# FraPria/proovread

Hardware: AMD Instinct MI355X
Metric: corrected long-read Mbases/sec per node (higher is better)
Workload: dtype int32

## Files before the change

### proovread_amd/csrc/seed_api.cpp

```cpp
#include <algorithm>
#include <climits>
#include <cstdio>
#include <cstdlib>
#include <cstring>
#include <vector>

#include "ctx.h"
#include "seed_index_dev.h"
#include "seed_plan.h"

static int seed_text4(pr_ctx *c, seedc::IndexView &v, hipStream_t s) {
    int rc = c->sd[SI_TEXT4].ensure((size_t)ix_pack4_words(v.n_text) * 8);
    if (rc) return rc;
    const int e = ix_pack4_launch(v.text, v.n_text, c->sd[SI_TEXT4].as<uint64_t>(), s);
    if (e) return set_error(PR_ERR_HIP, "text packing: %s", hipGetErrorString((hipError_t)e));
    v.text4 = c->sd[SI_TEXT4].as<uint64_t>();
    v.walk_nw = v.n_text > ((int64_t)64 << 24) ? 1 : 4;
    if (const char *w = getenv("PRGPU_SEED_WALK_NW"))
        v.walk_nw = atoi(w) == 1 ? 1 : 4;
    return 0;
}

static int upload_blk_fr(pr_ctx *c, seedc::IndexView &v, const int64_t *cstart, const int64_t *off, int n_lr,
                         int64_t l_pac, int64_t n_text, hipStream_t s) {
// ... 241 lines not shown
    seed_digest_tables(text, koff, kpos, kext, cnt, cstart, cblk, lro, ksplit, out6);
    return 0;
}

extern "C" int pr_seed_gpu_index_koff(pr_ctx *c, uint64_t *koff, uint64_t *ksplit) {
    if (!c || !koff) return set_error(PR_ERR_ARG, "null arg");
    if (!c->seed_loaded) return set_error(PR_ERR_ARG, "no device seed index");
    HIPCHK(hipSetDevice(c->device));
    HIPCHK(hipStreamSynchronize(c->stream));
    HIPCHK(hipMemcpy(koff, c->seed_view.koff, ((size_t)seedc::NK + 1) * 8, hipMemcpyDeviceToHost));
    if (ksplit && c->seed_view.ksplit)
        HIPCHK(hipMemcpy(ksplit, c->seed_view.ksplit, (size_t)seedc::NK * 8, hipMemcpyDeviceToHost));
    return 0;
}

extern "C" int pr_seed_gpu_index_last_ms(pr_ctx *c, double *ms) {
    if (!c || !ms) return set_error(PR_ERR_ARG, "null arg");
    *ms = c->ms_index;
    return 0;
}

extern "C" int pr_srset_load(pr_ctx *c, int64_t n_sr, const int64_t *off, const uint8_t *seq) {
    if (!c || n_sr < 0 || !off || (off[n_sr] && !seq) || off[0] != 0) return set_error(PR_ERR_ARG, "bad arg");
    HIPCHK(hipSetDevice(c->device));
    int rc = upload(c->ls[LS_SRSEQ], seq, (size_t)off[n_sr], c->stream);
    if (rc) return rc;
    HIPCHK(hipStreamSynchronize(c->stream));
    c->ss_off.assign(off, off + n_sr + 1);
    c->ss_samp_off.clear();
    c->ls[LS_SRSAMP].release();
    return 0;
}

static int gather_ranges(pr_ctx *c, const int64_t *ranges, int n_ranges, int64_t max_reads, DevBuf &dst,
                         std::vector<int64_t> &off) {
    if (c->ss_off.empty()) return set_error(PR_ERR_ARG, "no resident short reads (pr_srset_load)");
    const int64_t N = (int64_t)c->ss_off.size() - 1;
    off.assign(1, 0);
    for (int k = 0; k < n_ranges; ++k) {
        const int64_t r0 = ranges[2 * k], r1 = ranges[2 * k + 1];
        if (r0 < 0 || r1 < r0 || r1 > N) return set_error(PR_ERR_ARG, "record range outside the short reads");
        for (int64_t i = r0; i < r1; ++i) off.push_back(off.back() + c->ss_off[(size_t)i + 1] - c->ss_off[(size_t)i]);
    }
    if ((int64_t)off.size() - 1 > max_reads) return set_error(PR_ERR_CAPACITY, "too many short reads in one sample");
    HIPCHK(hipSetDevice(c->device));
    int rc = dst.ensure((size_t)off.back() + 1);
    if (rc) return rc;
    std::vector<int64_t> so, dn, ln;
    int64_t at = 0;
    for (int k = 0; k < n_ranges; ++k) {
        const int64_t b0 = c->ss_off[(size_t)ranges[2 * k]], b1 = c->ss_off[(size_t)ranges[2 * k + 1]];
        if (b1 > b0) {
            if (!so.empty() && so.back() + ln.back() == b0) ln.back() += b1 - b0;
            else so.push_back(b0), dn.push_back(at), ln.push_back(b1 - b0);
        }
        at += b1 - b0;
    }
    const int e = sr_gather_launch(c->ls[LS_SRSEQ].as<uint8_t>(), dst.as<uint8_t>(), so.data(), dn.data(), ln.data(),
                                   (int64_t)so.size(), (void *)c->stream);
    if (e) return set_error(PR_ERR_HIP, "short-read gather: %s", hipGetErrorString((hipError_t)e));
    return 0;
}

extern "C" int pr_srset_sample(pr_ctx *c, const int64_t *ranges, int n_ranges) {
    if (!c || n_ranges < 0 || (n_ranges && !ranges)) return set_error(PR_ERR_ARG, "null arg");
    std::vector<int64_t> off;
    int rc = gather_ranges(c, ranges, n_ranges, INT64_MAX, c->ls[LS_SRSAMP], off);
    if (rc) return rc;
    c->ss_samp_off.swap(off);
    return 0;
}

namespace {

struct SeedMap {
    pr_ctx *c;
    hipStream_t s;
    DevBuf *D;
    int n_sr;
    int qmax;
    SeedDev K;
    seedc::Caps small, caps;
    int64_t waves;
    int64_t lanes2;
    int64_t chunk;
    int32_t budget;
    std::vector<int32_t> nout, st;
    std::vector<int64_t> pre;
    int64_t total = 0, bad = 0;
    int32_t bad_flags = 0;
};

void map_plan(SeedMap &M, const pr_seed_opts *o, const int64_t *sr_off) {
    pr_ctx *c = M.c;
    int qmax = 1;
    for (int i = 0; i < M.n_sr; ++i) qmax = std::max<int>(qmax, (int)(sr_off[i + 1] - sr_off[i]));
    M.qmax = qmax;
    seedc::Caps &caps = M.caps, &small = M.small;
    caps = seedc::device_caps(qmax);
    caps.hi = c->seed_view.ksplit != nullptr;
    caps.nopos = 1;
    small = seedc::device_caps_small(std::min(qmax, caps.lmax));
    small.hi = caps.hi;
    small.nopos = 1;
    small.lazy = seedc::lazy_occ(*o) ? 1 : 0;
    if (const char *sc = getenv("PRGPU_SEED_SMALL"))
        sscanf(sc, "%d,%d,%d,%d,%d", &small.hits, &small.iv, &small.mems, &small.seeds, &small.chains);
    M.budget = small.lazy ? seedp::PASS1_LAZY_BUDGET : 0;
    if (const char *bu = getenv("PRGPU_SEED_BUDGET")) M.budget = small.lazy ? std::max(0, atoi(bu)) : 0;
    SeedDev &K = M.K;
    K = SeedDev{};
    K.V = c->seed_view;
    K.O = *o;
    K.n_sr = M.n_sr;
    K.caps = small;
    K.stride = seedc::scratch_bytes(small);
    const char *wpc = getenv("PRGPU_SEED_WAVES_PER_CU");
    size_t fr = 0, tot = 0;
    (void)hipMemGetInfo(&fr, &tot);
    (void)hipGetLastError();
    const int per_cu = wpc ? atoi(wpc) : 16;
    const int64_t full = caps.hi ? 0 : (int64_t)c->n_cu * per_cu * 64 * K.stride;
    M.waves = seedp::pass1_waves(M.n_sr, c->n_cu, per_cu, getenv("PRGPU_SEED_BALANCE") != nullptr,
                                 seedp::pass1_budget((int64_t)fr, (int64_t)M.D[SB_SCRATCH].cap, full), K.stride);
    K.n_lanes = M.waves;
    M.lanes2 = (int64_t)c->n_cu * seed_slots_per_cu(c->seed_view.walk_nw);
    const char *ob = getenv("PRGPU_SEED_OUT_MB");
    M.chunk = seedp::out_chunk(ob ? std::max<int64_t>(1, atoll(ob)) << 20
                                  : seedp::out_budget((int64_t)fr, (int64_t)M.D[SB_OUT].cap),
                               (int64_t)caps.out * (int64_t)sizeof(pr_seed_task));
}

int map_buffers(SeedMap &M, const pr_seed_opts *o, const uint8_t *sr_seq, bool in_sb_seq, const int64_t *sr_off) {
    pr_ctx *c = M.c;
    DevBuf *D = M.D;
    SeedDev &K = M.K;
    const int n_sr = M.n_sr;
    hipStream_t s = M.s;
    int rc;
    K.dp = nullptr;
    if (seedc::seed_flt_min_score(*o, M.qmax) >= 0) {
        if ((rc = D[SB_DP].ensure((size_t)M.waves * 2 * 201 * 64 * sizeof(int16_t)))) return rc;
        K.dp = D[SB_DP].as<int16_t>();
    }
    const int64_t scratch = std::max<int64_t>(M.waves * 64 * K.stride, M.lanes2 * seedc::scratch_bytes(M.caps));
    const int64_t nb = n_sr ? sr_off[n_sr] : 0;
    const int64_t slot_bytes = (int64_t)M.caps.out * (int64_t)sizeof(pr_seed_task);
    c->seed_sr_bases = nb;
    if ((!in_sb_seq && (rc = upload(D[SB_SEQ], sr_seq, (size_t)nb, s))) || (rc = upload(D[SB_OFF], sr_off, (size_t)n_sr + 1, s)) ||
        (rc = D[SB_SCRATCH].ensure((size_t)scratch)) ||
        (rc = D[SB_OUT].ensure((size_t)(std::min<int64_t>(M.chunk, n_sr) * slot_bytes + 16))) ||
        (rc = D[SB_NOUT].ensure((size_t)n_sr * 4 + 16)) || (rc = D[SB_STATUS].ensure((size_t)n_sr * 4 + 16)) ||
        (rc = D[SB_NEXT].ensure(256)) || (rc = D[SB_PRE].ensure(((size_t)n_sr + 1) * 8)) ||
        (rc = D[SB_DENSE].ensure(sizeof(pr_seed_task))))
        return rc;
    K.sr_seq = D[SB_SEQ].as<uint8_t>();
    K.sr_off = D[SB_OFF].as<int64_t>();
    K.out = D[SB_OUT].as<pr_seed_task>();
    K.n_out = D[SB_NOUT].as<int32_t>();
    K.status = D[SB_STATUS].as<int32_t>();
    K.next = D[SB_NEXT].as<int32_t>();
    K.prof = reinterpret_cast<unsigned long long *>(D[SB_NEXT].as<uint8_t>() + 64);
    HIPCHK(hipMemsetAsync(K.next, 0, 256, s));
    return 0;
}

int pass1(SeedMap &M, int64_t r0, int64_t r1, std::vector<int32_t> &redo, seedp::Flagged &f) {
    DevBuf *D = M.D;
    SeedDev &K = M.K;
    hipStream_t s = M.s;
    int rc;
    K.caps = M.small;
    K.caps.budget = M.budget;
    K.stride = seedc::scratch_bytes(M.small);
    K.n_lanes = M.waves;
    K.batch = 64;
    K.scratch = D[SB_SCRATCH].as<uint8_t>();
    K.rlist = nullptr;
    K.n_list = 0;
    K.out0 = r0;
    K.n_sr = r1;
    int32_t start = (int32_t)r0;
    const char *lpt = getenv("PRGPU_SEED_LPT");
    if (lpt && lpt[0] == '1') {
        int32_t *order = nullptr;
        if ((rc = D[SB_ORDER].ensure(seed_order_bytes(r1 - r0)))) return rc;
        int eo = seed_order_launch(K, r0, r1 - r0, D[SB_ORDER].p, &order, (void *)s);
        if (eo) return set_error(PR_ERR_HIP, "seed order: %s", hipGetErrorString((hipError_t)eo));
        K.rlist = order;
        K.n_list = r1 - r0;
        start = 0;
    }
    HIPCHK(hipMemcpyAsync(K.next, &start, 4, hipMemcpyHostToDevice, s));
    int e = seed_batch_launch(K, (void *)s);
    if (e) return set_error(PR_ERR_HIP, "seed kernel: %s", hipGetErrorString((hipError_t)e));
    if (r0 == 0) HIPCHK(hipEventRecord(M.c->ev[10], s));
    std::vector<int32_t> st1((size_t)(r1 - r0)), no1((size_t)(r1 - r0));
    if ((rc = download(st1.data(), D[SB_STATUS], (size_t)(r1 - r0), s, (size_t)r0)) ||
        (rc = download(no1.data(), D[SB_NOUT], (size_t)(r1 - r0), s, (size_t)r0)))
        return rc;
    HIPCHK(hipStreamSynchronize(s));
    for (int64_t i = r0; i < r1; ++i)
        if (st1[(size_t)(i - r0)]) {
            redo.push_back((int32_t)i);
            f.add(st1[(size_t)(i - r0)], no1[(size_t)(i - r0)]);
        }
    return 0;
}

int launch_pass(SeedMap &M, const char *name, bool by_wave, const seedc::Caps &caps, int64_t lanes,
                const std::vector<int32_t> &reads, int batch = 64) {
    SeedDev &K = M.K;
    K.caps = caps;
    K.stride = seedc::scratch_bytes(caps);
    K.n_lanes = lanes;
    K.batch = batch;
    K.scratch = M.D[SB_SCRATCH].as<uint8_t>();
    K.rlist = M.D[SB_PRE].as<int32_t>();
    K.n_list = (int64_t)reads.size();
    HIPCHK(hipMemcpyAsync(M.D[SB_PRE].p, reads.data(), reads.size() * 4, hipMemcpyHostToDevice, M.s));
    HIPCHK(hipMemsetAsync(K.next, 0, 4, M.s));
    const int e = by_wave ? seed_launch(K, (void *)M.s) : seed_batch_launch(K, (void *)M.s);
    if (e) return set_error(PR_ERR_HIP, "seed kernel (%s): %s", name, hipGetErrorString((hipError_t)e));
    return 0;
}

int still_flagged(SeedMap &M, int64_t r0, int64_t r1, const std::vector<int32_t> &reads, std::vector<int32_t> &left,
                  int32_t &flags) {
    std::vector<int32_t> st((size_t)(r1 - r0));
    int rc = download(st.data(), M.D[SB_STATUS], (size_t)(r1 - r0), M.s, (size_t)r0);
    if (rc) return rc;
    HIPCHK(hipStreamSynchronize(M.s));
    left.clear();
    flags = 0;
    for (int32_t i : reads)
        if (st[(size_t)(i - r0)]) left.push_back(i), flags |= st[(size_t)(i - r0)];
    return 0;
}

int pass1b(SeedMap &M, int64_t r0, int64_t r1, const seedp::Flagged &f, std::vector<int32_t> &redo, seedc::Caps &p2caps,
           bool &p2_ran) {
    if (!seedp::pass1b_wanted(f)) return 0;
    const seedp::Pass1bCaps p = seedp::pass1b_caps(M.small, M.caps, f);
    DevBuf &scr = M.D[SB_SCRATCH];
    int rc;
    size_t fr = 0, tot = 0;
    (void)hipMemGetInfo(&fr, &tot);
    (void)hipGetLastError();
    if (const int64_t want = seedp::pass1b_scratch_want(M.waves, f.n, p.sb, (int64_t)fr, (int64_t)scr.cap)) {
        HIPCHK(hipStreamSynchronize(M.s));
        if ((rc = scr.ensure((size_t)want))) return rc;
    }
    const char *p1b = getenv("PRGPU_SEED_1B");
    const seedp::Pass1bForce force =
        !p1b ? seedp::P1B_AUTO : !strcmp(p1b, "wave") ? seedp::P1B_FORCE_WAVE : seedp::P1B_FORCE_LANE;
    const seedp::Pass1bRun r =
        seedp::pass1b_run(p, f, M.small.hits, force, (int64_t)scr.cap, M.waves, M.lanes2, M.c->n_cu);
    if (r.mode == seedp::P1B_SKIP) return 0;
    const bool by_wave = r.mode == seedp::P1B_WAVE;
    seedp::Pass1bBatch b{64, r.wb};
    if (!by_wave && p.cb.lazy) {
        const char *bb = getenv("PRGPU_SEED_1B_BATCH");
        b = seedp::pass1b_batch(r, f.n, M.waves, (int64_t)scr.cap, p.sb, bb ? atoi(bb) : 0);
    }
    if ((rc = launch_pass(M, by_wave ? "pass 1b, waves" : "pass 1b", by_wave, by_wave ? p.cw : p.cb, by_wave ? r.ww : b.waves,
                          redo, b.batch)))
        return rc;
    M.c->seed_pass_reads[by_wave ? 1 : 0] += (int64_t)redo.size();
    if (by_wave) p2caps = p.cw, p2_ran = true;
    std::vector<int32_t> left;
    int32_t fl;
    if ((rc = still_flagged(M, r0, r1, redo, left, fl))) return rc;
    redo.swap(left);
    M.K.rlist = nullptr;
    M.K.n_list = 0;
    return 0;
}

int pass2_and_later(SeedMap &M, int64_t r0, int64_t r1, std::vector<int32_t> &redo, seedc::Caps cg, bool p2_ran) {
    if (redo.empty()) return 0;
    int rc;
    if (!p2_ran) {
        if ((rc = launch_pass(M, "pass 2", true, M.caps, std::min<int64_t>(M.lanes2, (int64_t)redo.size()), redo))) return rc;
        HIPCHK(hipStreamSynchronize(M.s));
        M.c->seed_pass_reads[2] += (int64_t)redo.size();
    }
    for (int pass = 3; pass <= 6; ++pass) {
        std::vector<int32_t> again;
        int32_t fl;
        if ((rc = still_flagged(M, r0, r1, redo, again, fl))) return rc;
        if (again.empty() || (fl & (seedc::SC_OVER_LEN | seedc::SC_OVER_OUT))) break;
        cg = seedc::grow_caps(cg, fl, 4);
        redo.swap(again);
        const int64_t lanes = std::min<int64_t>(M.lanes2, (int64_t)redo.size());
        if ((rc = M.D[SB_SCRATCH].ensure((size_t)(lanes * seedc::scratch_bytes(cg))))) return rc;
        char name[16];
        snprintf(name, sizeof name, "pass %d", pass);
        if ((rc = launch_pass(M, name, true, cg, lanes, redo))) return rc;
        HIPCHK(hipStreamSynchronize(M.s));
// ... 185 lines not shown
```

### proovread_amd/csrc/seed_core.h

```cpp
#pragma once
#include <math.h>
#include <stdint.h>

#include "../../include/prgpu.h"

#if defined(__HIPCC__)
#define SC_HD __host__ __device__ inline
#else
#define SC_HD inline
#endif

#if defined(PR_SEED_STATS) && !defined(__HIP_DEVICE_COMPILE__)
extern unsigned long long pr_seed_stat_g[24];
#define SC_STAT(k, v) __atomic_fetch_add(&pr_seed_stat_g[k], (unsigned long long)(v), __ATOMIC_RELAXED)
#else
#define SC_STAT(k, v) ((void)0)
#endif

namespace prgpu {
namespace seedc {

constexpr int KI = 12;
constexpr uint32_t NK = 1u << (2 * KI);
constexpr int KX = 28;
// ... 1179 lines not shown
    for (int ci = 0; ci < nch; ++ci) {
        const Chain &c = S.ch[ci];
        if (c.kept == 0) continue;
        const bool rev = S.seeds[c.head].rbeg >= I.l_pac;
        const int64_t L = I.lr_off[c.rid + 1] - I.lr_off[c.rid];
        const int64_t cs = rev ? I.l_pac + (I.l_pac - I.lr_off[c.rid + 1]) : I.lr_off[c.rid];
        if (no + c.n > cap_out) return SC_OVER_OUT;
        const int first = no;
        int idx = 0;
        int64_t r0 = INT64_MAX, r1 = INT64_MIN;
        for (int32_t k = c.head; k >= 0; k = S.seeds[k].nx) {
            const Seed &s = S.seeds[k];
            int score = s.len;
            if (flt >= 0) {
                const int x = scores ? scores[k]
                                     : (dp16 ? seed_sw_score(I, O, q, len, s, c.rid, dp16, dp16 + 201 * 64, 64)
                                             : seed_sw_score(I, O, q, len, s, c.rid, swH, swE));
                if (x >= 0 && x < flt) continue;
                score = x < 0 ? s.len * O.a : x;
            }
            const int64_t b = s.rbeg - (s.qbeg + cal_max_gap(O, s.qbeg));
            const int64_t e = s.rbeg + s.len + ((len - s.qbeg - s.len) + cal_max_gap(O, len - s.qbeg - s.len));
            r0 = r0 < b ? r0 : b;
            r1 = r1 > e ? r1 : e;
            pr_seed_task &t = out[no];
            t.sr = sid;
            t.lr = c.rid;
            t.strand = rev ? 1 : 0;
            t.qbeg = s.qbeg;
            t.rbeg = (int32_t)(s.rbeg - cs);
            t.slen = s.len;
            t.chain = nkept;
            t.rmax0 = score;
            t.rank = idx++;
            int j = no - 1;
            while (j >= first && (out[j].rmax0 < t.rmax0 || (out[j].rmax0 == t.rmax0 && out[j].rank < t.rank))) --j;
            const pr_seed_task v = t;
            for (int m = no; m > j + 1; --m) out[m] = out[m - 1];
            out[j + 1] = v;
            ++no;
        }
        if (no == first) continue;
        r0 -= cs;
        r1 -= cs;
        for (int m = first; m < no; ++m) {
            out[m].rank = m - first;
            out[m].rmax0 = (int32_t)(r0 > 0 ? r0 : 0);
            out[m].rmax1 = (int32_t)(r1 < L ? r1 : L);
        }
        ++nkept;
    }
    *n_out = no;
    SC_STAT(14, nch);
    SC_STAT(15, no);
    SC_TICK(5);
    return 0;
}

template <bool LZ = false>
SC_HD int map_after_occ(const IndexView &I, const pr_seed_opts &O, Scratch &S, const uint8_t *q, int len, int sid,
                        pr_seed_task *out, int cap_out, int *n_out, unsigned long long *ticks = nullptr,
                        const uint32_t *lcnt = nullptr, int16_t *dp16 = nullptr) {
    *n_out = 0;
    int nch = 0;
    const int err = map_chains<LZ>(I, O, S, q, len, &nch, ticks, lcnt);
    if (err) return err;
    return map_output(I, O, S, q, len, sid, nch, out, cap_out, n_out, nullptr, ticks, dp16);
}
#undef SC_TICK

SC_HD int map_read(const IndexView &I, const pr_seed_opts &O, Scratch &S, const uint8_t *q, int len, int sid,
                   pr_seed_task *out, int cap_out, int *n_out) {
    *n_out = 0;
    if (S.hend) {
        const int err = build_starts(I, S, q, len);
        return err ? err : map_after_occ<true>(I, O, S, q, len, sid, out, cap_out, n_out);
    }
    const int err = build_occ(I, S, q, len);
    return err ? err : map_after_occ<false>(I, O, S, q, len, sid, out, cap_out, n_out);
}

SC_HD bool lazy_occ(const pr_seed_opts &O) { return O.min_seed_len >= 17; }

}
}

namespace prgpu {
namespace seedc {

struct Caps {
    int32_t lmax, hits, iv, mems, seeds, chains, out;
    int32_t hi;
    int32_t nopos;
    int32_t lazy;
    int32_t budget;
};
SC_HD int device_out_cap(int qmax) { return qmax > 192 ? 2 * ((qmax + 15) & ~15) : 384; }
SC_HD Caps device_caps(int qmax = 0) {
    Caps c{1024, 8192, 256, 1024, 8192, 4096, 384, 0};
    c.out = device_out_cap(qmax);
    if (qmax > 192) {
        const int l = (qmax + 15) & ~15;
        c.hits = c.hits > 48 * l ? c.hits : 48 * l;
        c.iv = c.iv > l / 2 ? c.iv : l / 2;
        c.mems = c.mems > 2 * l ? c.mems : 2 * l;
        c.seeds = c.seeds > 4 * l ? c.seeds : 4 * l;
        c.chains = c.chains > 2 * l ? c.chains : 2 * l;
    }
    return c;
}
SC_HD Caps device_caps_small(int lmax) {
    const int l = lmax < 16 ? 16 : (lmax + 15) & ~15;
    Caps c{l, 4096, 64, 512, 512, 384, device_out_cap(lmax), 0};
    if (l > 160) {
        c.hits = c.hits > 24 * l ? c.hits : 24 * l;
        c.iv = c.iv > l / 4 ? c.iv : l / 4;
        c.mems = c.mems > 2 * l ? c.mems : 2 * l;
        c.seeds = c.seeds > 2 * l ? c.seeds : 2 * l;
        c.chains = c.chains > l ? c.chains : l;
    }
    return c;
}
SC_HD Caps grow_caps(Caps c, int32_t flags, int32_t hits_factor) {
    if (flags & SC_OVER_HITS) c.hits *= hits_factor;
    if (flags & SC_OVER_IV) c.iv *= 2;
    if (flags & SC_OVER_MEMS) c.mems *= 2;
    if (flags & SC_OVER_SEEDS) c.seeds *= 2;
    if (flags & SC_OVER_CHAINS) c.chains *= 2;
    return c;
}

SC_HD int64_t align8(int64_t x) { return (x + 7) & ~(int64_t)7; }
SC_HD int32_t range_table_size(int32_t chains) {
    int32_t h = 64;
    while (h < 2 * chains) h <<= 1;
    return h;
}

SC_HD int64_t scratch_bytes(const Caps &c) {
    int64_t b = 0;
    b += align8(4 * (int64_t)(c.lmax + 1));
    b += align8(8 * (int64_t)(c.lmax + 1));
    b += align8(4 * (int64_t)(c.lmax + 1));
    b += align8(4 * (int64_t)c.lmax * HB);
    if (!c.nopos) b += align8(4 * (int64_t)c.hits);
    b += align8(2 * (int64_t)c.hits);
    b += align8((int64_t)sizeof(Iv) * c.mems);
    b += 3 * align8((int64_t)sizeof(Iv) * c.iv);
    b += align8((int64_t)sizeof(Seed) * c.seeds);
    b += 2 * align8((int64_t)sizeof(Chain) * c.chains);
    b += 2 * align8(4 * (int64_t)c.chains);
    b += align8((int64_t)sizeof(RangeEnt) * range_table_size(c.chains));
    b = (b + 63) & ~(int64_t)63;
    b += align8((int64_t)sizeof(RangeRec) * c.chains);
    b += align8(2 * (int64_t)(c.lmax + 1) * RK);
    b += align8(8 * (int64_t)c.hits);
    if (c.hi && !c.nopos) b += align8((int64_t)c.hits);
    if (c.lazy) {
        b += align8(4 * (int64_t)(c.lmax + 1));
        b += align8((int64_t)(c.lmax + 1));
        b += align8(8 * (int64_t)(c.lmax / 16 + 4));
        b += align8(16);
    }
    return (b + 63) & ~(int64_t)63;
}

// ... 48 lines not shown
```

### proovread_amd/csrc/seed_dev.h

```cpp
#pragma once
#include <stdint.h>

#include <vector>

#include "seed_core.h"

namespace prgpu {

struct SeedDev {
    seedc::IndexView V;
    pr_seed_opts O;
    const uint8_t *sr_seq;
    const int64_t *sr_off;
    int64_t n_sr;
    uint8_t *scratch;
    int64_t stride;
    int64_t n_lanes;
    int32_t *next;
    unsigned long long *prof;
    seedc::Caps caps;
    pr_seed_task *out;
    int64_t out0;
    int32_t *n_out;
    int32_t *status;
    int16_t *dp;
    const int32_t *rlist;
    int64_t n_list;
    int32_t batch;
};

int seed_launch(const SeedDev &D, void *stream);
int seed_batch_launch(const SeedDev &D, void *stream);
size_t seed_order_bytes(int64_t n);
int seed_order_launch(const SeedDev &D, int64_t r0, int64_t n, void *buf, int32_t **order, void *stream);
constexpr int GATHER_RANGES = 112;
int sr_gather_launch(const uint8_t *src, uint8_t *dst, const int64_t *s_off, const int64_t *d_off, const int64_t *len,
                     int64_t n, void *stream);
int seed_slots_per_cu(int walk_nw);
int seed_compact_launch(const pr_seed_task *slots, const int32_t *n_out, const int64_t *pre, int64_t n_sr, int cap,
                        pr_seed_task *out, void *stream);

seedc::IndexView seed_index_view(const pr_seed_index *h);
struct SeedIndexSizes {
    int64_t text, cstart, cblk, lr_off, koff, kpos, ksplit, cnt[seedc::KI - 1];
};
SeedIndexSizes seed_index_sizes(const pr_seed_index *h);
void seed_digest_tables(const std::vector<uint8_t> &text, const std::vector<uint64_t> &koff,
                        const std::vector<uint32_t> &kpos, const std::vector<uint64_t> &kext,
                        const std::vector<std::vector<uint32_t>> &cnt, const std::vector<int64_t> &cstart,
                        const std::vector<int32_t> &cblk, const std::vector<int64_t> &lr_off,
                        const std::vector<uint64_t> &ksplit, uint64_t *out6);

}
```

### proovread_amd/csrc/seed_kernels.hip

```cpp
#include <hip/hip_runtime.h>

#include <rocprim/device/device_radix_sort.hpp>

#include "seed_core.h"
#include "seed_dev.h"

namespace prgpu {

#ifndef SEED_WAVES_DEF
#define SEED_WAVES_DEF 4
#endif
#ifndef SEED_LMAX_DEF
#define SEED_LMAX_DEF 1024
#endif
constexpr int SEED_WAVES = SEED_WAVES_DEF;
constexpr int SEED_LMAX = SEED_LMAX_DEF;
#ifndef SEED_MINB
#define SEED_MINB 4
#endif
#ifndef SEED_WAVE_MINB
#define SEED_WAVE_MINB SEED_MINB
#endif
#ifndef OCC_U
#define OCC_U 2
// ... 679 lines not shown
            }
            if (len > 0 && !err) {
                const seedc::Occ occ{&D.V, &S, q, len, lcnt};
                nm = seedc::collect_intv(occ, S, D.O, q, len, err, D.prof ? pl : nullptr);
            }
            if (D.prof) atomicMax(&D.prof[18], wall_clock64() - tm);
        }
        err = __shfl(err, 0, 64);
        nm = __shfl(nm, 0, 64);
        if (len > 0 && !err) {
            const unsigned long long tc = D.prof && lane == 0 ? wall_clock64() : 0ULL;
            __threadfence_block();
            int ncv = chain_wave(D.V, D.O, S, nm, lane, ho);
            unsigned long long tf = D.prof && lane == 0 ? wall_clock64() : 0ULL;
            if (lane == 0 && D.prof) atomicAdd(&D.prof[14 + (ncv == -1 ? 1 : 0)], tf - tc);
            if (ncv == -2) {
                ncv = 0;
                err = seedc::SC_OVER_CHAINS;
            }
            if (lane == 0 && ncv == -1) {
                ncv = 0;
                err = seedc::chain_seq(D.V, D.O, S, nm, &ncv);
                if (D.prof) {
                    const unsigned long long t_ = wall_clock64();
                    atomicAdd(&D.prof[13], 1ULL);
                    atomicAdd(&D.prof[15], t_ - tf);
                    tf = t_;
                }
            }
            err = __shfl(err, 0, 64);
            ncv = __shfl(ncv, 0, 64);
            __threadfence_block();
            wave_sync_lds();
            bool flt = err != 0 || chain_flt_wave(D.O, S, ncv, lane, &nch);
            if (lane == 0) {
                if (!flt) seedc::chain_flt(D.O, S, ncv, &nch);
                if (D.prof) {
                    const unsigned long long t_ = wall_clock64();
                    pl[3] += t_ - tc;
                    atomicAdd(&D.prof[16], t_ - tf);
                }
                if (!err && seedc::seed_flt_min_score(D.O, len) >= 0 && 3 * S.cap_seeds <= 2 * S.cap_hits &&
                    2 * 201 * 64 * 2 <= 4 * S.lmax * seedc::HB)
                    nlist = seedc::flt_seed_list(S, nch, (int32_t *)S.hfr + S.cap_seeds, S.cap_seeds);
            }
        }
        err = __shfl(err, 0, 64);
        nlist = __shfl(nlist, 0, 64);
        if (nlist > 0) {
            __threadfence_block();
            const int32_t *list = (const int32_t *)S.hfr + S.cap_seeds;
            int32_t *rid = (int32_t *)S.hfr + 2 * S.cap_seeds;
            if (lane == 0) {
                int x = 0;
                for (int ci = 0; ci < nch; ++ci) {
                    const seedc::Chain &c = S.ch[ci];
                    if (c.kept == 0) continue;
                    for (int32_t k = c.head; k >= 0; k = S.seeds[k].nx) rid[x++] = c.rid;
                }
            }
            __threadfence_block();
            int32_t *scores = (int32_t *)S.hfr;
            int16_t *H = (int16_t *)S.ge + lane, *E = H + 201 * 64;
            for (int x = lane; x < nlist; x += 64) {
                const int32_t k = list[x];
                scores[k] = seedc::seed_sw_score(D.V, D.O, q, len, S.seeds[k], rid[x], H, E, 64);
            }
            __threadfence_block();
        }
        if (lane == 0) {
            int n = 0;
            if (len > 0 && !err)
                err = seedc::map_output(D.V, D.O, S, q, len, i, nch, D.out + (int64_t)(i - D.out0) * D.caps.out,
                                        D.caps.out, &n, nlist >= 0 ? (const int32_t *)S.hfr : nullptr,
                                        D.prof ? pl : nullptr);
            D.n_out[i] = err ? 0 : n;
            D.status[i] = err;
            if (D.prof) atomicMax(&D.prof[19], wall_clock64() - t0);
        }
        __threadfence_block();
    }
}

template <bool LZ>
__global__ void __launch_bounds__(64 * SEED_WAVES, SEED_MINB) seed_batch_kernel(SeedDev D) {
    __shared__ __attribute__((aligned(16))) int32_t hoff_lds[SEED_WAVES][SEED_LMAX + 4];
    __shared__ uint64_t q4_lds[SEED_WAVES][SEED_LMAX / 16 + 4];
    __shared__ uint32_t lcnt[seedc::LC_N];
    load_lcnt(D.V, lcnt);
    const int lane = threadIdx.x & 63, wv = threadIdx.x >> 6;
    const int64_t slot = (int64_t)blockIdx.x * SEED_WAVES + wv;
    if (slot >= D.n_lanes) return;
    int batch = 64;
    if constexpr (LZ) batch = D.batch;
    uint8_t *base = D.scratch + slot * batch * D.stride;
    int32_t *ho = hoff_lds[wv];
    unsigned long long pt[2] = {0ULL, 0ULL};
    unsigned long long lt[6] = {0ULL, 0ULL, 0ULL, 0ULL, 0ULL, 0ULL};
    unsigned long long ot[3] = {0ULL, 0ULL, 0ULL};
    constexpr bool HTAB_REUSE = LZ;
    if (HTAB_REUSE) {
        struct __attribute__((aligned(8))) Ent2 { seedc::RangeEnt a, b; };
        const seedc::Scratch S0 = seedc::carve(base, D.caps);
        const int64_t off = reinterpret_cast<uint8_t *>(S0.htab) - base;
        const Ent2 free2{{-1, -1}, {-1, -1}};
        for (int rd = 0; rd < batch; ++rd) {
            Ent2 *t = reinterpret_cast<Ent2 *>(base + (int64_t)rd * D.stride + off);
            for (int k = lane; k < S0.hsize / 2; k += 64) t[k] = free2;
        }
        __threadfence_block();
        wave_sync_lds();
    }
    for (;;) {
        int b0 = 0;
        if (lane == 0) b0 = atomicAdd(D.next, batch);
        b0 = __shfl(b0, 0, 64);
        const int64_t nlim = D.rlist ? D.n_list : D.n_sr;
        if (b0 >= nlim) {
            if (D.prof) {
#pragma unroll
                for (int k = 0; k < 6; ++k)
                    for (int o = 32; o > 0; o >>= 1) lt[k] += __shfl_xor(lt[k], o, 64);
            }
            if (D.prof && lane == 0) {
                atomicAdd(&D.prof[0], pt[0]);
                atomicAdd(&D.prof[1], pt[1]);
                for (int k = 0; k < 6; ++k) atomicAdd(&D.prof[4 + k], lt[k]);
                for (int k = 0; k < 3; ++k) atomicAdd(&D.prof[10 + k], ot[k]);
            }
            break;
        }
        const unsigned long long t0 = D.prof ? wall_clock64() : 0ULL;
        int my_err = 0, my_hits = 0;
        const int nb = (int)(nlim - b0 < batch ? nlim - b0 : batch);
        for (int rd = 0; rd < nb; ++rd) {
            const int i = D.rlist ? D.rlist[b0 + rd] : b0 + rd;
            const int64_t o = D.sr_off[i];
            const int len = (int)(D.sr_off[i + 1] - o);
            seedc::Scratch S = seedc::carve(base + (int64_t)rd * D.stride, D.caps);
            int err = 0, nh = 0;
            if (len > S.lmax || len > SEED_LMAX - 1) err = seedc::SC_OVER_LEN;
            if (len > 0 && !err)
                err = build_occ_wave<4>(D.V, S, D.sr_seq + o, len, ho, lane, q4_lds[wv], lcnt, &nh, D.prof ? ot : nullptr,
                                     LZ);
            if (lane == rd) my_err = err, my_hits = nh;
        }
        const unsigned long long t1 = D.prof ? wall_clock64() : 0ULL;
        if (lane < nb) {
            const int i = D.rlist ? D.rlist[b0 + lane] : b0 + lane;
            const int64_t o = D.sr_off[i];
            const int len = (int)(D.sr_off[i + 1] - o);
            seedc::Scratch S = seedc::carve(base + (int64_t)lane * D.stride, D.caps);
            S.htab_clean = HTAB_REUSE;
            int n = 0, err = my_err;
            if (len > 0 && !err)
                err = seedc::map_after_occ<LZ>(D.V, D.O, S, D.sr_seq + o, len, i, D.out + (int64_t)(i - D.out0) * D.caps.out,
                                           D.caps.out, &n, D.prof ? lt : nullptr, lcnt,
                                           D.dp ? D.dp + slot * (2 * 201 * 64) + lane : nullptr);
            D.n_out[i] = (my_err & seedc::SC_OVER_HITS) ? -my_hits
                         : (LZ && (err & seedc::SC_OVER_HITS)) ? -S.lz[2]
                                                                        : (err ? 0 : n);
            D.status[i] = err;
        }
        if (D.prof && lane == 0) {
            pt[0] += t1 - t0;
            pt[1] += wall_clock64() - t1;
        }
        __threadfence_block();
    }
}

__global__ void __launch_bounds__(256) seed_cost_kernel(seedc::IndexView V, const uint8_t *sr_seq, const int64_t *sr_off,
                                                        int64_t r0, int64_t n, uint32_t *key, int32_t *val) {
    for (int64_t k = (int64_t)blockIdx.x * blockDim.x + threadIdx.x; k < n; k += (int64_t)gridDim.x * blockDim.x) {
        const int64_t i = r0 + k;
        const int64_t o = sr_off[i];
        const int len = (int)(sr_off[i + 1] - o);
        uint32_t code = 0u, cost = 0u;
        int valid = 0;
        for (int p = 0; p < len; ++p) {
            const uint32_t c = sr_seq[o + p];
            if (c > 3u) {
                valid = 0;
                continue;
            }
            code = ((code << 2) | c) & (seedc::NK - 1u);
            if (++valid >= seedc::KI && (p & 1) == 0) {
                const uint64_t m = V.koff[code + 1] - V.koff[code];
                cost += m < 1024u ? (uint32_t)m : 1024u;
            }
        }
        key[k] = 0xFFFFFFFFu - cost;
        val[k] = (int32_t)i;
    }
}
size_t seed_order_bytes(int64_t n) {
    size_t tb = 0;
    (void)rocprim::radix_sort_pairs(nullptr, tb, (uint32_t *)nullptr, (uint32_t *)nullptr, (int32_t *)nullptr,
                                    (int32_t *)nullptr, (size_t)(n > 0 ? n : 1), 0u, 32u, (hipStream_t)0);
    return (size_t)(n > 0 ? n : 1) * 16 + ((tb + 255) & ~(size_t)255) + 256;
}
int seed_order_launch(const SeedDev &D, int64_t r0, int64_t n, void *buf, int32_t **order, void *stream) {
    hipStream_t s = (hipStream_t)stream;
    const size_t n1 = (size_t)(n > 0 ? n : 1);
    uint32_t *k0 = (uint32_t *)buf, *k1 = k0 + n1;
    int32_t *v0 = (int32_t *)(k1 + n1), *v1 = v0 + n1;
    void *temp = (void *)(((uintptr_t)(v1 + n1) + 255) & ~(uintptr_t)255);
    size_t tb = 0;
    (void)rocprim::radix_sort_pairs(nullptr, tb, k0, k1, v0, v1, n1, 0u, 32u, s);
    int64_t grid = (n + 255) / 256;
    grid = grid < 4096 ? (grid > 0 ? grid : 1) : 4096;
    hipLaunchKernelGGL(seed_cost_kernel, dim3((unsigned)grid), dim3(256), 0, s, D.V, D.sr_seq, D.sr_off, r0, n, k0, v0);
    hipError_t e = hipGetLastError();
    if (e != hipSuccess) return (int)e;
    if ((e = rocprim::radix_sort_pairs(temp, tb, k0, k1, v0, v1, (size_t)n, 0u, 32u, s)) != hipSuccess) return (int)e;
    *order = v1;
    return 0;
}

struct GatherArgs {
    int64_t s_off[GATHER_RANGES], d_off[GATHER_RANGES], len[GATHER_RANGES];
};
constexpr int64_t GATHER_TILE = 64 << 10;
__global__ void __launch_bounds__(256) sr_gather_kernel(const uint8_t *__restrict__ src, uint8_t *__restrict__ dst, GatherArgs A) {
    const int64_t n = A.len[blockIdx.y];
    const uint8_t *s = src + A.s_off[blockIdx.y];
    uint8_t *d = dst + A.d_off[blockIdx.y];
    const int64_t head = std::min<int64_t>(n, (int64_t)((16 - (reinterpret_cast<uintptr_t>(d) & 15)) & 15));
    if (blockIdx.x == 0)
        for (int64_t k = threadIdx.x; k < head; k += blockDim.x) d[k] = s[k];
    const int64_t body = (n - head) & ~(int64_t)15;
    for (int64_t t0 = (int64_t)blockIdx.x * GATHER_TILE; t0 < body; t0 += (int64_t)gridDim.x * GATHER_TILE) {
        const int64_t t1 = std::min<int64_t>(body, t0 + GATHER_TILE);
        for (int64_t k = t0 + (int64_t)threadIdx.x * 16; k < t1; k += (int64_t)blockDim.x * 16) {
            uint4 v;
            __builtin_memcpy(&v, s + head + k, 16);
            *reinterpret_cast<uint4 *>(d + head + k) = v;
        }
    }
    if (blockIdx.x == 0)
        for (int64_t k = head + body + threadIdx.x; k < n; k += blockDim.x) d[k] = s[k];
}
int sr_gather_launch(const uint8_t *src, uint8_t *dst, const int64_t *s_off, const int64_t *d_off, const int64_t *len,
                     int64_t n, void *stream) {
    for (int64_t k0 = 0; k0 < n; k0 += GATHER_RANGES) {
        const int m = (int)std::min<int64_t>(GATHER_RANGES, n - k0);
        GatherArgs A{};
        int64_t lmax = 0;
        for (int k = 0; k < m; ++k) {
            A.s_off[k] = s_off[k0 + k];
            A.d_off[k] = d_off[k0 + k];
            A.len[k] = len[k0 + k];
            lmax = std::max(lmax, A.len[k]);
        }
        const int64_t tiles = std::max<int64_t>(1, std::min<int64_t>(256, (lmax + GATHER_TILE - 1) / GATHER_TILE));
        hipLaunchKernelGGL(sr_gather_kernel, dim3((unsigned)tiles, (unsigned)m), dim3(256), 0, (hipStream_t)stream, src, dst, A);
        const hipError_t e = hipGetLastError();
        if (e != hipSuccess) return (int)e;
    }
    return 0;
}

int seed_slots_per_cu(int walk_nw) {
    int nb = 0;
    const hipError_t e = walk_nw == 1 ? hipOccupancyMaxActiveBlocksPerMultiprocessor(&nb, seed_wave_kernel<1>, 64 * SEED_WAVES, 0)
                                      : hipOccupancyMaxActiveBlocksPerMultiprocessor(&nb, seed_wave_kernel<4>, 64 * SEED_WAVES, 0);
    if (e != hipSuccess || nb < 1)
        nb = 2;
    return nb * SEED_WAVES;
}

int seed_launch(const SeedDev &D, void *stream) {
    if (D.n_list <= 0) return 0;
    const int64_t blocks = (D.n_lanes + SEED_WAVES - 1) / SEED_WAVES;
    if (D.V.walk_nw == 1)
        hipLaunchKernelGGL(seed_wave_kernel<1>, dim3((unsigned)blocks), dim3(64 * SEED_WAVES), 0, (hipStream_t)stream, D);
    else
        hipLaunchKernelGGL(seed_wave_kernel<4>, dim3((unsigned)blocks), dim3(64 * SEED_WAVES), 0, (hipStream_t)stream, D);
    return (int)hipGetLastError();
}

int seed_batch_launch(const SeedDev &D, void *stream) {
    if (D.n_sr <= 0) return 0;
    if (D.caps.lazy && (D.batch < 1 || D.batch > 64)) return (int)hipErrorInvalidValue;
    const int64_t blocks = (D.n_lanes + SEED_WAVES - 1) / SEED_WAVES;
    if (D.caps.lazy)
        hipLaunchKernelGGL(seed_batch_kernel<true>, dim3((unsigned)blocks), dim3(64 * SEED_WAVES), 0, (hipStream_t)stream, D);
    else
        hipLaunchKernelGGL(seed_batch_kernel<false>, dim3((unsigned)blocks), dim3(64 * SEED_WAVES), 0, (hipStream_t)stream, D);
    return (int)hipGetLastError();
}

__global__ void seed_compact_kernel(const pr_seed_task *slots, const int32_t *n_out, const int64_t *pre, int64_t n_sr,
                                    int cap, pr_seed_task *out) {
    const int64_t i = ((int64_t)blockIdx.x * blockDim.x + threadIdx.x) >> 6;
    const int lane = threadIdx.x & 63;
    if (i >= n_sr) return;
    const int n = n_out[i];
    constexpr int TW = (int)(sizeof(pr_seed_task) / 4);
    const uint32_t *src = reinterpret_cast<const uint32_t *>(slots + i * cap);
    uint32_t *dst = reinterpret_cast<uint32_t *>(out + pre[i]);
    for (int k = lane; k < n * TW; k += 64) dst[k] = src[k];
}

int seed_compact_launch(const pr_seed_task *slots, const int32_t *n_out, const int64_t *pre, int64_t n_sr, int cap,
                        pr_seed_task *out, void *stream) {
    if (n_sr <= 0) return 0;
    const int64_t blocks = (n_sr + 3) / 4;
    hipLaunchKernelGGL(seed_compact_kernel, dim3((unsigned)blocks), dim3(256), 0, (hipStream_t)stream, slots, n_out, pre,
                       n_sr, cap, out);
    return (int)hipGetLastError();
}

}
```

### proovread_amd/csrc/seed_plan.h

```cpp
#pragma once
#include <stdint.h>

#include <algorithm>

#include "seed_core.h"

namespace prgpu {
namespace seedp {

inline int64_t scratch_budget(int64_t free_bytes, int64_t have) {
    return std::min<int64_t>((int64_t)40 << 30, std::max<int64_t>((int64_t)24 << 30, (free_bytes + have) * 15 / 100));
}
inline bool scratch_growth_fits(int64_t want, int64_t free_bytes, int64_t have) { return want <= (free_bytes + have) / 2; }

inline int64_t pass1_budget(int64_t free_bytes, int64_t have, int64_t full) {
    const int64_t b = scratch_budget(free_bytes, have);
    return full > b && full <= ((int64_t)40 << 30) && full <= (free_bytes + have) / 4 ? full : b;
}
inline int64_t pass1_wave_cap(int n_cu, int64_t budget, int64_t stride) {
    return std::max<int64_t>(n_cu, budget / (64 * stride));
}
inline int64_t pass1_waves(int64_t n_sr, int n_cu, int waves_per_cu, bool balance, int64_t budget, int64_t stride) {
    int64_t waves = (int64_t)n_cu * waves_per_cu;
    const int64_t nbatch = (n_sr + 63) / 64;
    if (waves > nbatch) waves = nbatch;
    if (waves < 1) waves = 1;
    if (balance) {
        const int64_t rounds = (nbatch + waves - 1) / waves;
        waves = (nbatch + rounds - 1) / rounds;
    }
    return std::min(waves, pass1_wave_cap(n_cu, budget, stride));
}

constexpr int32_t PASS1_LAZY_BUDGET = 0;

inline int64_t out_budget(int64_t free_bytes, int64_t have) {
    return std::min<int64_t>((int64_t)16 << 30, std::max<int64_t>((int64_t)8 << 30, (free_bytes + have) / 10));
}
inline int64_t out_chunk(int64_t out_budget, int64_t slot_bytes) {
    return std::max<int64_t>(64, out_budget / slot_bytes / 64 * 64);
}

struct Flagged {
    int64_t n = 0;
    int32_t flags = 0;
    int64_t need_max = 0, need_sum = 0, need_n = 0;
    void add(int32_t status, int32_t n_out) {
        ++n;
        flags |= status;
        need_max = std::max<int64_t>(need_max, -(int64_t)n_out);
        if (n_out < 0) need_sum -= n_out, ++need_n;
    }
};

inline bool pass1b_wanted(const Flagged &f) { return f.n > 4096 && !(f.flags & (seedc::SC_OVER_LEN | seedc::SC_OVER_OUT)); }

struct Pass1bCaps {
    seedc::Caps cb;
    seedc::Caps cw;
    int64_t sb, sw;
};
inline Pass1bCaps pass1b_caps(const seedc::Caps &small, const seedc::Caps &caps, const Flagged &f) {
    Pass1bCaps p;
    p.cb = small;
    if (f.flags & seedc::SC_OVER_HITS) {
        p.cb.hits = (int32_t)std::min<int64_t>(
            std::max<int64_t>((int64_t)p.cb.hits + 512, (f.need_max + f.need_max / 8 + 511) & ~(int64_t)511), (int64_t)1 << 20);
        const int64_t g = std::min<int64_t>(16, std::max<int64_t>(1, p.cb.hits / small.hits));
        p.cb.chains = (int32_t)(p.cb.chains * g);
        p.cb.seeds = (int32_t)(p.cb.seeds * g);
    }
    p.cb = seedc::grow_caps(p.cb, f.flags, 1);
    p.cw = caps;
    p.cw.hits = std::max(caps.hits, p.cb.hits);
    p.cw.iv = std::max(caps.iv, p.cb.iv);
    p.cw.mems = std::max(caps.mems, p.cb.mems);
    p.cw.seeds = std::max(caps.seeds, p.cb.seeds);
    p.cw.chains = std::max(caps.chains, p.cb.chains);
    p.sb = seedc::scratch_bytes(p.cb);
    p.sw = seedc::scratch_bytes(p.cw);
    return p;
}
inline int64_t pass1b_scratch_want(int64_t waves, int64_t n_flagged, int64_t sb, int64_t free_bytes, int64_t have) {
    const int64_t want = std::min<int64_t>(waves, (n_flagged + 63) / 64) * 64 * sb;
    return want > have && want <= scratch_budget(free_bytes, have) && scratch_growth_fits(want, free_bytes, have) ? want : 0;
}

enum Pass1bMode { P1B_SKIP, P1B_LANE, P1B_WAVE };
enum Pass1bForce { P1B_AUTO, P1B_FORCE_LANE, P1B_FORCE_WAVE };
struct Pass1bRun {
    bool by_wave;
    int64_t wb;
    int64_t ww;
    Pass1bMode mode;
};
inline Pass1bRun pass1b_run(const Pass1bCaps &p, const Flagged &f, int32_t small_hits, Pass1bForce force, int64_t scratch_cap,
                            int64_t waves, int64_t lanes2, int n_cu) {
    Pass1bRun r;
    r.wb = std::min<int64_t>(std::min<int64_t>(scratch_cap / (64 * p.sb), (f.n + 63) / 64), waves);
    r.by_wave = force != P1B_AUTO ? force == P1B_FORCE_WAVE : f.need_sum > 4 * (int64_t)small_hits * f.need_n;
    r.ww = std::min<int64_t>(std::min<int64_t>(lanes2, f.n), scratch_cap / p.sw);
    r.mode = !pass1b_wanted(f) ? P1B_SKIP : r.by_wave && r.ww >= n_cu ? P1B_WAVE : r.wb >= n_cu ? P1B_LANE : P1B_SKIP;
    return r;
}

struct Pass1bBatch {
    int32_t batch;
    int64_t waves;
};
inline Pass1bBatch pass1b_batch(const Pass1bRun &r, int64_t n_flagged, int64_t waves, int64_t scratch_cap, int64_t sb,
                                int force) {
    Pass1bBatch b;
    waves = std::max<int64_t>(waves, 1);
    const int64_t per = force > 0 ? force : (n_flagged + waves - 1) / waves;
// ... 9 lines not shown
```

Baseline: 231.1.

## Size pass-1 batch slices to spread reads across all waves, add guided dequeue

Pass 1 of the seed kernel used to pull fixed batches of 64 reads per wave, with the wave count computed separately. It now picks a per-wave slice count from the read count and wave budget, with a floor of 16, so more waves get work and the tail shrinks. Scratch is sized by slices instead of 64. An optional guided dequeue, where the batch size shrinks as work runs out, and an equal-split rule are added behind an environment variable. A templated fast path keeps the original constant batch of 64. Smaller batches mean more atomic dequeues and more per-wave hash-table setup.

```diff
diff --git a/proovread_amd/csrc/seed_api.cpp b/proovread_amd/csrc/seed_api.cpp
--- a/proovread_amd/csrc/seed_api.cpp
+++ b/proovread_amd/csrc/seed_api.cpp
@@ -347,6 +347,9 @@
     SeedDev K;
     seedc::Caps small, caps;
     int64_t waves;
+    int32_t slices;
+    seedp::Pass1Rule rule;
+    int floor, force;
     int64_t lanes2;
     int64_t chunk;
     int32_t budget;
@@ -386,14 +389,32 @@
     (void)hipGetLastError();
     const int per_cu = wpc ? atoi(wpc) : 16;
     const int64_t full = caps.hi ? 0 : (int64_t)c->n_cu * per_cu * 64 * K.stride;
-    M.waves = seedp::pass1_waves(M.n_sr, c->n_cu, per_cu, getenv("PRGPU_SEED_BALANCE") != nullptr,
-                                 seedp::pass1_budget((int64_t)fr, (int64_t)M.D[SB_SCRATCH].cap, full), K.stride);
-    K.n_lanes = M.waves;
-    M.lanes2 = (int64_t)c->n_cu * seed_slots_per_cu(c->seed_view.walk_nw);
     const char *ob = getenv("PRGPU_SEED_OUT_MB");
     M.chunk = seedp::out_chunk(ob ? std::max<int64_t>(1, atoll(ob)) << 20
                                   : seedp::out_budget((int64_t)fr, (int64_t)M.D[SB_OUT].cap),
                                (int64_t)caps.out * (int64_t)sizeof(pr_seed_task));
+    M.rule = seedp::PASS1_RULE;
+    M.floor = seedp::PASS1_FLOOR;
+    M.force = 0;
+    if (const char *dq = getenv("PRGPU_SEED_DEQUEUE")) {
+        if (dq[0] == 'G' || dq[0] == 'g') M.rule = seedp::P1_GUIDED;
+        if (dq[0] == 'E' || dq[0] == 'e') M.rule = seedp::P1_EQUAL;
+        if (dq[0] == 'S' || dq[0] == 's') M.rule = seedp::P1_SLICES;
+        if (const char *fl = strchr(dq, ',')) M.floor = std::min(64, std::max(1, atoi(fl + 1)));
+    }
+    if (const char *fb = getenv("PRGPU_SEED_BATCH")) M.force = std::min(64, std::max(0, atoi(fb)));
+    const int64_t budget1 = seedp::pass1_budget((int64_t)fr, (int64_t)M.D[SB_SCRATCH].cap, full);
+    if (getenv("PRGPU_SEED_BALANCE")) {
+        M.waves = seedp::pass1_waves(M.n_sr, c->n_cu, per_cu, true, budget1, K.stride);
+        M.slices = 64;
+    } else {
+        const seedp::Pass1Spread sp =
+            seedp::pass1_spread(std::min<int64_t>(M.chunk, M.n_sr), c->n_cu, per_cu, budget1, K.stride, M.floor, M.force);
+        M.waves = sp.waves;
+        M.slices = sp.slices;
+    }
+    K.n_lanes = M.waves;
+    M.lanes2 = (int64_t)c->n_cu * seed_slots_per_cu(c->seed_view.walk_nw);
 }
 
 int map_buffers(SeedMap &M, const pr_seed_opts *o, const uint8_t *sr_seq, bool in_sb_seq, const int64_t *sr_off) {
@@ -408,7 +429,7 @@
         if ((rc = D[SB_DP].ensure((size_t)M.waves * 2 * 201 * 64 * sizeof(int16_t)))) return rc;
         K.dp = D[SB_DP].as<int16_t>();
     }
-    const int64_t scratch = std::max<int64_t>(M.waves * 64 * K.stride, M.lanes2 * seedc::scratch_bytes(M.caps));
+    const int64_t scratch = std::max<int64_t>(M.waves * M.slices * K.stride,M.lanes2 * seedc::scratch_bytes(M.caps));
     const int64_t nb = n_sr ? sr_off[n_sr] : 0;
     const int64_t slot_bytes = (int64_t)M.caps.out * (int64_t)sizeof(pr_seed_task);
     c->seed_sr_bases = nb;
@@ -439,7 +460,11 @@
     K.caps.budget = M.budget;
     K.stride = seedc::scratch_bytes(M.small);
     K.n_lanes = M.waves;
-    K.batch = 64;
+    const seedp::Pass1Dequeue dq = seedp::pass1_dequeue(r1 - r0, M.slices, M.waves, M.rule, M.floor, M.force);
+    K.slices = M.slices;
+    K.batch = dq.batch;
+    K.dq_rule = dq.rule;
+    K.dq_floor = dq.floor;
     K.scratch = D[SB_SCRATCH].as<uint8_t>();
     K.rlist = nullptr;
     K.n_list = 0;
@@ -479,7 +504,9 @@
     K.caps = caps;
     K.stride = seedc::scratch_bytes(caps);
     K.n_lanes = lanes;
-    K.batch = batch;
+    K.slices = K.batch = batch;
+    K.dq_rule = seedc::DQ_CONST;
+    K.dq_floor = 1;
     K.scratch = M.D[SB_SCRATCH].as<uint8_t>();
     K.rlist = M.D[SB_PRE].as<int32_t>();
     K.n_list = (int64_t)reads.size();
diff --git a/proovread_amd/csrc/seed_core.h b/proovread_amd/csrc/seed_core.h
--- a/proovread_amd/csrc/seed_core.h
+++ b/proovread_amd/csrc/seed_core.h
@@ -1285,6 +1285,20 @@
 
 SC_HD bool lazy_occ(const pr_seed_opts &O) { return O.min_seed_len >= 17; }
 
+enum { DQ_CONST = 0, DQ_GUIDED = 1 };
+SC_HD int dequeue_want(int rule, int batch, int floor, int slices, int64_t left, int64_t waves) {
+    int want = batch;
+    if (rule == DQ_GUIDED) {
+        const uint32_t l = left < 0 ? 0u : left > INT32_MAX ? (uint32_t)INT32_MAX : (uint32_t)left;
+        const uint32_t w = waves < 1 ? 1u : waves > INT32_MAX ? (uint32_t)INT32_MAX : (uint32_t)waves;
+        const uint32_t share = l / w + (l % w ? 1u : 0u);
+        want = share > 64u ? 64 : (int)share;
+        want = want < floor ? floor : want;
+    }
+    want = want > slices ? slices : want;
+    return want < 1 ? 1 : want;
+}
+
 }
 }
 
diff --git a/proovread_amd/csrc/seed_dev.h b/proovread_amd/csrc/seed_dev.h
--- a/proovread_amd/csrc/seed_dev.h
+++ b/proovread_amd/csrc/seed_dev.h
@@ -26,7 +26,10 @@
     int16_t *dp;
     const int32_t *rlist;
     int64_t n_list;
+    int32_t slices;
     int32_t batch;
+    int32_t dq_rule;
+    int32_t dq_floor;
 };
 
 int seed_launch(const SeedDev &D, void *stream);
diff --git a/proovread_amd/csrc/seed_kernels.hip b/proovread_amd/csrc/seed_kernels.hip
--- a/proovread_amd/csrc/seed_kernels.hip
+++ b/proovread_amd/csrc/seed_kernels.hip
@@ -785,8 +785,9 @@
     }
 }
 
-template <bool LZ>
+template <bool LZ, bool B64 = false>
 __global__ void __launch_bounds__(64 * SEED_WAVES, SEED_MINB) seed_batch_kernel(SeedDev D) {
+    static_assert(!(LZ && B64), "the lazy kernel takes its dequeue size from the launch");
     __shared__ __attribute__((aligned(16))) int32_t hoff_lds[SEED_WAVES][SEED_LMAX + 4];
     __shared__ uint64_t q4_lds[SEED_WAVES][SEED_LMAX / 16 + 4];
     __shared__ uint32_t lcnt[seedc::LC_N];
@@ -794,9 +795,8 @@
     const int lane = threadIdx.x & 63, wv = threadIdx.x >> 6;
     const int64_t slot = (int64_t)blockIdx.x * SEED_WAVES + wv;
     if (slot >= D.n_lanes) return;
-    int batch = 64;
-    if constexpr (LZ) batch = D.batch;
-    uint8_t *base = D.scratch + slot * batch * D.stride;
+    const int slices = B64 ? 64 : D.slices;
+    uint8_t *base = D.scratch + slot * slices * D.stride;
     int32_t *ho = hoff_lds[wv];
     unsigned long long pt[2] = {0ULL, 0ULL};
     unsigned long long lt[6] = {0ULL, 0ULL, 0ULL, 0ULL, 0ULL, 0ULL};
@@ -807,7 +807,7 @@
         const seedc::Scratch S0 = seedc::carve(base, D.caps);
         const int64_t off = reinterpret_cast<uint8_t *>(S0.htab) - base;
         const Ent2 free2{{-1, -1}, {-1, -1}};
-        for (int rd = 0; rd < batch; ++rd) {
+        for (int rd = 0; rd < slices; ++rd) {
             Ent2 *t = reinterpret_cast<Ent2 *>(base + (int64_t)rd * D.stride + off);
             for (int k = lane; k < S0.hsize / 2; k += 64) t[k] = free2;
         }
@@ -815,11 +815,19 @@
         wave_sync_lds();
     }
     for (;;) {
-        int b0 = 0;
-        if (lane == 0) b0 = atomicAdd(D.next, batch);
-        b0 = __shfl(b0, 0, 64);
         const int64_t nlim = D.rlist ? D.n_list : D.n_sr;
-        if (b0 >= nlim) {
+        unsigned *ctr = reinterpret_cast<unsigned *>(D.next);
+        int want = seedc::dequeue_want(seedc::DQ_CONST, B64 ? 64 : D.batch, 0, slices, 0, 1);
+        if (!B64 && D.dq_rule == seedc::DQ_GUIDED) {
+            if (lane == 0)
+                want = seedc::dequeue_want(seedc::DQ_GUIDED, D.batch, D.dq_floor, slices,
+                                           nlim - (int64_t)__atomic_load_n(ctr, __ATOMIC_RELAXED), D.n_lanes);
+            want = __shfl(want, 0, 64);
+        }
+        unsigned u0 = 0u;
+        if (lane == 0) u0 = atomicAdd(ctr, (unsigned)want);
+        u0 = (unsigned)__shfl((int)u0, 0, 64);
+        if ((int64_t)u0 >= nlim) {
             if (D.prof) {
 #pragma unroll
                 for (int k = 0; k < 6; ++k)
@@ -835,7 +843,8 @@
         }
         const unsigned long long t0 = D.prof ? wall_clock64() : 0ULL;
         int my_err = 0, my_hits = 0;
-        const int nb = (int)(nlim - b0 < batch ? nlim - b0 : batch);
+        const int b0 = (int)u0;
+        const int nb = (int)(nlim - b0 < want ? nlim - b0 : want);
         for (int rd = 0; rd < nb; ++rd) {
             const int i = D.rlist ? D.rlist[b0 + rd] : b0 + rd;
             const int64_t o = D.sr_off[i];
@@ -985,10 +994,15 @@
 
 int seed_batch_launch(const SeedDev &D, void *stream) {
     if (D.n_sr <= 0) return 0;
-    if (D.caps.lazy && (D.batch < 1 || D.batch > 64)) return (int)hipErrorInvalidValue;
+    if (D.slices < 1 || D.slices > 64 || D.batch < 1 || D.batch > D.slices || D.dq_floor < 0 ||
+        (D.dq_rule != seedc::DQ_CONST && D.dq_rule != seedc::DQ_GUIDED))
+        return (int)hipErrorInvalidValue;
     const int64_t blocks = (D.n_lanes + SEED_WAVES - 1) / SEED_WAVES;
     if (D.caps.lazy)
         hipLaunchKernelGGL(seed_batch_kernel<true>, dim3((unsigned)blocks), dim3(64 * SEED_WAVES), 0, (hipStream_t)stream, D);
+    else if (D.slices == 64 && D.batch == 64 && D.dq_rule == seedc::DQ_CONST)
+        hipLaunchKernelGGL((seed_batch_kernel<false, true>), dim3((unsigned)blocks), dim3(64 * SEED_WAVES), 0,
+                           (hipStream_t)stream, D);
     else
         hipLaunchKernelGGL(seed_batch_kernel<false>, dim3((unsigned)blocks), dim3(64 * SEED_WAVES), 0, (hipStream_t)stream, D);
     return (int)hipGetLastError();
diff --git a/proovread_amd/csrc/seed_plan.h b/proovread_amd/csrc/seed_plan.h
--- a/proovread_amd/csrc/seed_plan.h
+++ b/proovread_amd/csrc/seed_plan.h
@@ -30,6 +30,50 @@
         waves = (nbatch + rounds - 1) / rounds;
     }
     return std::min(waves, pass1_wave_cap(n_cu, budget, stride));
+}
+
+enum Pass1Rule { P1_EQUAL, P1_GUIDED, P1_SLICES };
+constexpr Pass1Rule PASS1_RULE = P1_SLICES;
+constexpr int32_t PASS1_FLOOR = 16;
+
+struct Pass1Spread {
+    int32_t slices;
+    int64_t waves;
+};
+inline Pass1Spread pass1_spread(int64_t n, int n_cu, int waves_per_cu, int64_t budget, int64_t stride, int floor, int force) {
+    Pass1Spread p;
+    int64_t waves = std::max<int64_t>(1, (int64_t)n_cu * waves_per_cu);
+    waves = std::min(waves, pass1_wave_cap(n_cu, budget, stride));
+    const int64_t per = (std::max<int64_t>(n, 1) + waves - 1) / waves;
+    const int64_t fl = std::min<int64_t>(64, std::max<int64_t>(1, floor));
+    p.slices = (int32_t)(force > 0 ? std::min(64, force) : std::min<int64_t>(64, std::max(per, fl)));
+    p.waves = std::min(waves, std::max<int64_t>(1, (n + p.slices - 1) / p.slices));
+    return p;
+}
+
+struct Pass1Dequeue {
+    int32_t rule;
+    int32_t batch;
+    int32_t floor;
+};
+inline Pass1Dequeue pass1_dequeue(int64_t n, int32_t slices, int64_t waves, Pass1Rule rule, int floor, int force) {
+    Pass1Dequeue d;
+    waves = std::max<int64_t>(waves, 1);
+    n = std::max<int64_t>(n, 1);
+    d.floor = std::min(slices, std::max(1, floor));
+    d.rule = rule == P1_GUIDED && force <= 0 ? seedc::DQ_GUIDED : seedc::DQ_CONST;
+    if (force > 0) {
+        d.batch = std::min(slices, force);
+    } else if (rule == P1_SLICES) {
+        d.batch = slices;
+    } else if (rule == P1_GUIDED) {
+        d.batch = slices;
+    } else {
+        const int64_t rounds = (n + slices * waves - 1) / (slices * waves);
+        const int64_t batch = (n + rounds * waves - 1) / (rounds * waves);
+        d.batch = (int32_t)std::min<int64_t>(slices, std::max<int64_t>(batch, d.floor));
+    }
+    return d;
 }
 
 constexpr int32_t PASS1_LAZY_BUDGET = 0;
```

After: 233.3 (median of 3 runs). Within noise of the previous version (+1.0%).
